# nimiq/snark-setup-operator

Hardware: NVIDIA B200
Metric: phase1_contribute_points_per_s (higher is better)
Workload: dtype u32 limbs (Montgomery, integer pipe)

## Files before the change

### snark-setup-operator_b200/csrc/curve_ops.cuh

```cuda
#pragma once
#include <type_traits>
#include "host.cuh"
#include "kernels.cuh"
#include "msm.cuh"
#include "pairing.cuh"
#include "keygen.cuh"
#include "blake2b.h"
#include <cub/device/device_radix_sort.cuh>
#include <random>

namespace sso {

struct CurveOps {
  int (*tau_tables)(Ctx& c, int si, uint64_t first_index, const uint8_t* tau, const uint8_t* const coeffs[TAU_COEFF_SLOTS],
                    uint32_t** d_table, char* err, size_t errcap);
  int (*batch_exp)(Ctx& c, int si, uint32_t group, const VecBatch& batch, uint32_t in_compressed, const uint32_t* d_table,
                   uint32_t out_compressed, uint32_t check, uint32_t* d_status, char* err, size_t errcap);
  int (*batch_exp_chunk)(Ctx& c, int si, const VecBatch& b1, const VecBatch& b2, uint32_t in_compressed, const uint32_t* d_table,
                         uint32_t out_compressed, uint32_t check, uint32_t* d_status, char* err, size_t errcap);
  int (*reencode)(Ctx& c, int si, uint32_t group, const uint8_t* d_in, uint32_t in_compressed, uint64_t n, uint8_t* d_out,
                  uint32_t out_compressed, uint32_t check, uint32_t subgroup, uint32_t* d_aff, uint32_t* d_status, char* err,
                  size_t errcap);
  int (*msm_pairs)(Ctx& c, int si, uint32_t group, const uint32_t* d_aff_a, const uint32_t* d_aff_b, uint64_t n,
                   const uint8_t seed32[32], const uint64_t* tweak, uint8_t* d_out, char* err, size_t errcap);
// ... 16 lines not shown
  int (*fft_part_tables)(Ctx& c, int si, const uint32_t* root, uint32_t squarings, uint64_t e, const uint8_t* scale, uint32_t** d_table,
                         char* err, size_t errcap);
  int (*fft_row_stage)(Ctx& c, int si, uint32_t group, const uint8_t* d_x, uint64_t rows, uint64_t row_len, uint32_t log_ns, const uint32_t* root,
                       uint32_t two_adicity, uint32_t* d_status, uint8_t* d_out, char* err, size_t errcap);
};

template <class Fr>
__global__ void k_tau_tables(const uint32_t* tau_canon, const uint32_t* coeff_canon, uint64_t first_index, uint32_t* table) {
  uint32_t tid = blockIdx.x * blockDim.x + threadIdx.x;
  if (tid < (uint32_t)TAU_TABLE_ELEMS) body_tau_tables<Fr>(tid, tau_canon, coeff_canon, first_index, table);
}

#ifndef SSO_EXP_MIN_BLOCKS
#define SSO_EXP_MIN_BLOCKS 1
#endif
#ifndef SSO_EXP_MIN_BLOCKS_G1
#define SSO_EXP_MIN_BLOCKS_G1 SSO_EXP_MIN_BLOCKS
#endif
#ifndef SSO_EXP_MIN_BLOCKS_G2
#define SSO_EXP_MIN_BLOCKS_G2 SSO_EXP_MIN_BLOCKS
#endif
#ifndef SSO_SPLIT_GROUPS
#define SSO_SPLIT_GROUPS 0
#endif
template <class G>
__global__ void __launch_bounds__(128, (G::GROUP == 0 ? SSO_EXP_MIN_BLOCKS_G1 : SSO_EXP_MIN_BLOCKS_G2)) k_batch_exp(const __grid_constant__ VecBatch batch, uint32_t in_compressed,
                                                    const uint32_t* table, uint32_t check, uint32_t* jac_out, uint32_t* status) {
  extern __shared__ __align__(16) unsigned char tree_raw[];
  block_batch_exp<G>(blockIdx.x, batch, in_compressed, table, check, jac_out, status, reinterpret_cast<typename G::F::T*>(tree_raw));
}

template <class G>
__global__ void __launch_bounds__(128, 1) k_normalize_write(const __grid_constant__ VecBatch batch, const uint32_t* jac,
                                                          uint32_t out_compressed) {
  uint32_t tid = blockIdx.x * blockDim.x + threadIdx.x;
  body_normalize_write<G>(tid, batch, jac, out_compressed);
}

template <class GC>
__global__ void __launch_bounds__(128, 1) k_subgroup_coop(uint32_t n, const uint32_t* aff, const uint8_t* pts, uint32_t* status) {
  using CO = Coop<GC::F::DEG>;
  if (!CO::lane_active()) return;
  body_subgroup_coop<GC>(blockIdx.x * ExpBlock<GC>::PPB + CO::group_in_block(), n, aff, pts, status);
}

template <class G>
__global__ void __launch_bounds__(128, 1) k_reencode(uint32_t n, const uint8_t* in, uint32_t in_compressed, uint8_t* out,
                                                   uint32_t out_compressed, uint32_t check, uint32_t subgroup, uint32_t* aff_out,
                                                   uint32_t* status) {
  uint32_t tid = blockIdx.x * blockDim.x + threadIdx.x;
  body_reencode<G>(tid, n, in, in_compressed, out, out_compressed, check, subgroup, aff_out, status);
}

#ifndef SSO_CHUNK_MIN_BLOCKS
#define SSO_CHUNK_MIN_BLOCKS 1
#endif
template <class G1, class G2>
__global__ void __launch_bounds__(128, SSO_CHUNK_MIN_BLOCKS) k_batch_exp_chunk(const __grid_constant__ VecBatch b1, const __grid_constant__ VecBatch b2,
                                                          uint32_t nb2, uint32_t in_compressed, const uint32_t* table, uint32_t check,
                                                          uint32_t* jac1, uint32_t* jac2, uint32_t* status) {
  extern __shared__ __align__(16) unsigned char tree_raw[];
  if (blockIdx.x < nb2) {
    block_batch_exp<G2>(blockIdx.x, b2, in_compressed, table, check, jac2, status, reinterpret_cast<typename G2::F::T*>(tree_raw));
  } else {
    block_batch_exp<G1>(blockIdx.x - nb2, b1, in_compressed, table, check, jac1, status, reinterpret_cast<typename G1::F::T*>(tree_raw));
  }
}
template <class G1, class G2>
__global__ void __launch_bounds__(128, 1) k_normalize_chunk(const __grid_constant__ VecBatch b1, const __grid_constant__ VecBatch b2,
                                                          uint32_t nb2, const uint32_t* jac1, const uint32_t* jac2, uint32_t out_compressed) {
  if (blockIdx.x < nb2) body_normalize_write<G2>(blockIdx.x * blockDim.x + threadIdx.x, b2, jac2, out_compressed);
  else body_normalize_write<G1>((blockIdx.x - nb2) * blockDim.x + threadIdx.x, b1, jac1, out_compressed);
}

inline int coop_g2_override() {
  const char* e = getenv("SSO_COOP_G2");
  return !e || !e[0] ? -1 : (e[0] == '0' ? 0 : 1);
}
template <class GC> inline bool coop_g2_enabled() {
  int o = coop_g2_override();
  return o < 0 ? GC::COOP_DEFAULT : o != 0;
}

template <class G1, class G2>
inline int run_batch_exp_chunk(Ctx& c, int si, const VecBatch& b1, const VecBatch& b2, uint32_t in_compressed, const uint32_t* d_table,
                               uint32_t out_compressed, uint32_t check, uint32_t* d_status, char* err, size_t errcap) {
  uint64_t n1 = b1.total, n2 = b2.total;
  if (n1 + n2 == 0) return SSO_OK;
  for (uint32_t i = 0; i < b1.nseg; i++) if (b1.seg[i].n > (1u << 24)) { set_err(err, errcap, "vector longer than 2^24 elements: split the call"); return SSO_E_ARG; }
  for (uint32_t i = 0; i < b2.nseg; i++) if (b2.seg[i].n > (1u << 24)) { set_err(err, errcap, "vector longer than 2^24 elements: split the call"); return SSO_E_ARG; }
  cudaStream_t st = c.s[si];
  uint32_t *d_jac1 = nullptr, *d_jac2 = nullptr;
  int rc;
  if ((rc = c.alloc((void**)&d_jac1, (size_t)n1 * 3 * G1::F::WORDS * 4, si))) return rc;
  if ((rc = c.alloc((void**)&d_jac2, (size_t)n2 * 3 * G2::F::WORDS * 4, si))) return rc;
  uint32_t nb2 = div_up(n2, EXP_BLOCK), nb1 = div_up(n1, EXP_BLOCK);
  constexpr size_t TREE_BYTES = 16 + 2 * EXP_BLOCK * (sizeof(typename G1::F::T) > sizeof(typename G2::F::T) ? sizeof(typename G1::F::T)
                                                                                                             : sizeof(typename G2::F::T));
  if (TREE_BYTES > 48 * 1024)
    CUDA_TRY(cudaFuncSetAttribute(k_batch_exp_chunk<G1, G2>, cudaFuncAttributeMaxDynamicSharedMemorySize, (int)TREE_BYTES));
#if SSO_SPLIT_GROUPS
  {
    const int sj = (c.s[1] && !c.aliased) ? 1 : si;
    constexpr size_t TREE1 = 16 + 2 * EXP_BLOCK * sizeof(typename G1::F::T), TREE2 = 16 + 2 * EXP_BLOCK * sizeof(typename G2::F::T);
    if (TREE1 > 48 * 1024) CUDA_TRY(cudaFuncSetAttribute(k_batch_exp<G1>, cudaFuncAttributeMaxDynamicSharedMemorySize, (int)TREE1));
    if (TREE2 > 48 * 1024) CUDA_TRY(cudaFuncSetAttribute(k_batch_exp<G2>, cudaFuncAttributeMaxDynamicSharedMemorySize, (int)TREE2));
    if (sj != si && (rc = c.fork(si, sj))) return rc;
    if (n2) {
      c.begin(PK_BATCH_EXP_G2, si, n2);
      k_batch_exp<G2><<<nb2, EXP_BLOCK, TREE2, st>>>(b2, in_compressed, d_table, check, d_jac2, d_status);
      c.end(si);
// ... 640 lines not shown
```

### snark-setup-operator_b200/csrc/curves.cuh

```cuda
#pragma once
#include "ec.cuh"
#include "coop.cuh"

namespace sso {

using Fr253 = Fp<P_r253>;
using Fq377 = Fp<P_q377>;
using Fq761 = Fp<P_q761>;
using Fq4 = Fp<P_q4>;
using Fq6 = Fp<P_q6>;

using Fq377x2 = Fp2<Fq377, SmallNR<Fq377, 5, true>>;
using Fq4x2 = Fp2<Fq4, SmallNR<Fq4, 13, false>>;
using Fq6x3 = Fp3<Fq6, SmallNR<Fq6, 11, false>>;

static constexpr bool PRIME_ORDER_bls12_377_g1 = false, PRIME_ORDER_bls12_377_g2 = false, PRIME_ORDER_bw6_761_g1 = false,
                      PRIME_ORDER_bw6_761_g2 = false, PRIME_ORDER_mnt4_753_g1 = true, PRIME_ORDER_mnt4_753_g2 = false,
                      PRIME_ORDER_mnt6_753_g1 = true, PRIME_ORDER_mnt6_753_g2 = false;
#define SSO_GROUP_COMMON(NAME, FIELD, SCALAR)                                                      \
  using F = FIELD;                                                                                  \
  using Fr = SCALAR;                                                                                \
  __device__ __forceinline__ static typename F::T coeff_b() { return F::from_const(c_##NAME##_b); } \
  __device__ __forceinline__ static const uint32_t* order() { return c_##NAME##_order; }           \
  __device__ __forceinline__ static typename F::T gen_x() { return F::from_const(c_##NAME##_gx); }  \
  __device__ __forceinline__ static typename F::T gen_y() { return F::from_const(c_##NAME##_gy); }  \
  __device__ __forceinline__ static const uint32_t* cofactor() { return c_##NAME##_cofactor; }      \
  static constexpr int COFACTOR_WORDS = COFACTOR_WORDS_##NAME;                                     \
  static constexpr bool PRIME_ORDER = PRIME_ORDER_##NAME;

struct Bls12_377_G1 {
  static constexpr bool AFFINE_TABLE = true;
  static constexpr bool HAS_GLV = true;
  using Glv = GLV_bls12_377_g1;
  static constexpr int ENDO_SUBGROUP_TEST = 1;
  static constexpr bool HAS_GLS4 = false;
  static constexpr bool HAS_GLS2 = false;
  using Endo = ENDO_bls12_377;
  static constexpr uint32_t GROUP = 0;
  SSO_GROUP_COMMON(bls12_377_g1, Fq377, Fr253)
  static constexpr bool A_IS_ZERO = true;
  __device__ __forceinline__ static F::T mul_a(const F::T&) { return F::zero(); }
  __device__ __forceinline__ static bool field_sqrt(const F::T& a, F::T& o) { return F::sqrt(a, o); }
};
struct Bls12_377_G2 {
  static constexpr float VERIFY_WEIGHT = 1.6f;
  static constexpr bool AFFINE_TABLE = true;
  static constexpr bool HAS_GLV = true;
  using Glv = GLV_bls12_377_g2;
  static constexpr int ENDO_SUBGROUP_TEST = 2;
  static constexpr bool HAS_GLS4 = true;
  static constexpr bool HAS_GLS2 = false;
  using Endo = ENDO_bls12_377;
  static constexpr uint32_t GROUP = 1;
  SSO_GROUP_COMMON(bls12_377_g2, Fq377x2, Fr253)
  static constexpr bool A_IS_ZERO = true;
  __device__ __forceinline__ static F::T mul_a(const F::T&) { return F::zero(); }
  __device__ __forceinline__ static bool field_sqrt(const F::T& a, F::T& o) { return F::sqrt(a, o); }
};
struct Bw6_761_G1 {
  static constexpr bool AFFINE_TABLE = true;
  static constexpr bool HAS_GLV = true;
  using Glv = GLV_bw6_761_g1;
  static constexpr int ENDO_SUBGROUP_TEST = 3;
  using Endo = ENDO_bw6_761;
  static constexpr bool HAS_GLS4 = false;
  static constexpr bool HAS_GLS2 = false;
  static constexpr uint32_t GROUP = 0;
  SSO_GROUP_COMMON(bw6_761_g1, Fq761, Fq377)
  static constexpr bool A_IS_ZERO = true;
  __device__ __forceinline__ static F::T mul_a(const F::T&) { return F::zero(); }
  __device__ __forceinline__ static bool field_sqrt(const F::T& a, F::T& o) { return F::sqrt(a, o); }
};
struct Bw6_761_G2 {
  static constexpr float VERIFY_WEIGHT = 1.5f;
  static constexpr bool AFFINE_TABLE = true;
  static constexpr bool HAS_GLV = true;
  using Glv = GLV_bw6_761_g2;
  static constexpr int ENDO_SUBGROUP_TEST = 0;
  static constexpr bool HAS_GLS4 = false;
  static constexpr bool HAS_GLS2 = false;
  static constexpr uint32_t GROUP = 1;
  SSO_GROUP_COMMON(bw6_761_g2, Fq761, Fq377)
  static constexpr bool A_IS_ZERO = true;
  __device__ __forceinline__ static F::T mul_a(const F::T&) { return F::zero(); }
  __device__ __forceinline__ static bool field_sqrt(const F::T& a, F::T& o) { return F::sqrt(a, o); }
};
struct Mnt4_753_G1 {
  static constexpr bool AFFINE_TABLE = true;
  static constexpr bool HAS_GLV = false;
  static constexpr int ENDO_SUBGROUP_TEST = 0;
  static constexpr bool HAS_GLS4 = false;
  static constexpr bool HAS_GLS2 = false;
  static constexpr uint32_t GROUP = 0;
  SSO_GROUP_COMMON(mnt4_753_g1, Fq4, Fq6)
  static constexpr bool A_IS_ZERO = false;
  __device__ __forceinline__ static F::T mul_a(const F::T& x) { return F::dbl(x); }
  __device__ __forceinline__ static F::T mad_a_lazy(const F::T& c, const F::T& x) { return F::mad_small_lazy(c, 2u, x); }
  __device__ __forceinline__ static bool field_sqrt(const F::T& a, F::T& o) { return F::sqrt(a, o); }
};
struct Mnt4_753_G2 {
  static constexpr float VERIFY_WEIGHT = 10.f;
  static constexpr bool AFFINE_TABLE = true;
  static constexpr bool HAS_GLV = false;
  static constexpr int ENDO_SUBGROUP_TEST = 4;
  using Endo = ENDO_mnt4_753;
  static constexpr bool HAS_GLS4 = false;
  static constexpr bool HAS_GLS2 = true;
  static constexpr uint32_t GROUP = 1;
  SSO_GROUP_COMMON(mnt4_753_g2, Fq4x2, Fq6)
  static constexpr bool A_IS_ZERO = false;
  __device__ __forceinline__ static F::T mul_a(const F::T& x) { return F::mul_small<26>(x); }
  __device__ __forceinline__ static F::T mad_a_lazy(const F::T& c, const F::T& x) { return F::mad_small_lazy(c, 26u, x); }
  __device__ __forceinline__ static bool field_sqrt(const F::T& a, F::T& o) { return F::sqrt(a, o); }
};
struct Mnt6_753_G1 {
  static constexpr bool AFFINE_TABLE = true;
  static constexpr bool HAS_GLV = false;
  static constexpr int ENDO_SUBGROUP_TEST = 0;
  static constexpr bool HAS_GLS4 = false;
  static constexpr bool HAS_GLS2 = false;
  static constexpr uint32_t GROUP = 0;
  SSO_GROUP_COMMON(mnt6_753_g1, Fq6, Fq4)
  static constexpr bool A_IS_ZERO = false;
  __device__ __forceinline__ static F::T mul_a(const F::T& x) { return F::mul_small<11>(x); }
  __device__ __forceinline__ static F::T mad_a_lazy(const F::T& c, const F::T& x) { return F::mad_small_lazy(c, 11u, x); }
  __device__ __forceinline__ static bool field_sqrt(const F::T& a, F::T& o) { return F::sqrt(a, o); }
};
struct Mnt6_753_G2 {
  static constexpr float VERIFY_WEIGHT = 20.f;
  static constexpr bool AFFINE_TABLE = false;
  static constexpr bool HAS_GLV = false;
  static constexpr int ENDO_SUBGROUP_TEST = 4;
  using Endo = ENDO_mnt6_753;
  static constexpr bool HAS_GLS4 = false;
  static constexpr bool HAS_GLS2 = true;
  static constexpr uint32_t GROUP = 1;
  SSO_GROUP_COMMON(mnt6_753_g2, Fq6x3, Fq4)
  static constexpr bool A_IS_ZERO = false;
  __device__ __forceinline__ static F::T mul_a(const F::T& x) {
    return F::mul_small<11>(F::mul_u2(x));
  }
  __device__ __forceinline__ static F::T mad_a_lazy(const F::T& c, const F::T& x) { return F::add_lazy(c, mul_a(x)); }
  __device__ __forceinline__ static bool field_sqrt(const F::T& a, F::T& o) {
#ifdef SSO_FQ3_SQRT_PLAIN
    return F::sqrt_ts<TS_q6x3>(a, o, c_q6x3_tm1h, c_q6x3_tsz);
#else
    return F::sqrt_ts_norm<TS_q6x3>(a, o, c_q6x3_tsz, ENDO_mnt6_753::w1(), ENDO_mnt6_753::w2());
#endif
  }
};

#define SSO_GROUP_COOP(NAME, PLAIN, ...)                                                            \
  using Plain = PLAIN;                                                                              \
  using F = __VA_ARGS__;                                                                            \
  __device__ __forceinline__ static typename F::T coeff_b() { return F::from_const(c_##NAME##_b); } \
  __device__ __forceinline__ static bool field_sqrt(const typename F::T&, typename F::T&) { return false; }
struct Bls12_377_G2C : Bls12_377_G2 {
  static constexpr bool COOP_DEFAULT = false;
  SSO_GROUP_COOP(bls12_377_g2, Bls12_377_G2, CFp2<Fq377, 5, true>)
  __device__ __forceinline__ static F::T mul_a(const F::T&) { return F::zero(); }
};
struct Mnt4_753_G2C : Mnt4_753_G2 {
  static constexpr bool COOP_DEFAULT = true;
  SSO_GROUP_COOP(mnt4_753_g2, Mnt4_753_G2, CFp2<Fq4, 13, false>)
  __device__ __forceinline__ static F::T mul_a(const F::T& x) { return F::mul_small<26>(x); }
  __device__ __forceinline__ static F::T mad_a_lazy(const F::T& c, const F::T& x) { return F::mad_small_lazy(c, 26u, x); }
};
#ifndef SSO_MNT6_COOP_AFFINE
#define SSO_MNT6_COOP_AFFINE 1
#endif
struct Mnt6_753_G2C : Mnt6_753_G2 {
  static constexpr bool AFFINE_TABLE = SSO_MNT6_COOP_AFFINE != 0;
  static constexpr bool COOP_DEFAULT = true;
  SSO_GROUP_COOP(mnt6_753_g2, Mnt6_753_G2, CFp3<Fq6, 11, false>)
  __device__ __forceinline__ static F::T mul_a(const F::T& x) { return F::mul_small<11>(F::mul_u2(x)); }
  __device__ __forceinline__ static F::T mad_a_lazy(const F::T& c, const F::T& x) { return F::add_lazy(c, mul_a(x)); }
};
template <class G> struct CoopOf { using type = void; };
template <> struct CoopOf<Bls12_377_G2> { using type = Bls12_377_G2C; };
template <> struct CoopOf<Mnt4_753_G2> { using type = Mnt4_753_G2C; };
template <> struct CoopOf<Mnt6_753_G2> { using type = Mnt6_753_G2C; };

enum : uint32_t { CURVE_BLS12_377 = 0, CURVE_BW6_761 = 1, CURVE_MNT4_753 = 2, CURVE_MNT6_753 = 3 };
enum : uint32_t { GROUP_G1 = 0, GROUP_G2 = 1 };

template <class Fn> inline int dispatch_group(uint32_t curve, uint32_t group, Fn&& f) {
  switch (curve * 2 + group) {
    case 0: f(Bls12_377_G1{}); return 0;
    case 1: f(Bls12_377_G2{}); return 0;
    case 2: f(Bw6_761_G1{}); return 0;
    case 3: f(Bw6_761_G2{}); return 0;
    case 4: f(Mnt4_753_G1{}); return 0;
    case 5: f(Mnt4_753_G2{}); return 0;
    case 6: f(Mnt6_753_G1{}); return 0;
    case 7: f(Mnt6_753_G2{}); return 0;
  }
  return -1;
}

}
```

### snark-setup-operator_b200/csrc/ec.cuh

```cuda
#pragma once
#include "ext.cuh"

#ifndef SSO_POINT_BY_VALUE
#define SSO_POINT_BY_VALUE 0
#endif
#ifndef SSO_LAZY_EC
#define SSO_LAZY_EC 1
#endif

namespace sso {

template <class Cfg> struct SW {
  using F = typename Cfg::F;
  using FT = typename F::T;
  struct Affine { FT x, y; bool inf; };
  struct Jac { FT X, Y, Z; };

  __device__ __forceinline__ static Jac identity() { return Jac{F::one(), F::one(), F::zero()}; }
  __device__ __forceinline__ static bool is_identity(const Jac& p) { return F::is_zero(p.Z); }
  __device__ __forceinline__ static Jac from_affine(const Affine& a) {
    if (a.inf) return identity();
    return Jac{a.x, a.y, F::one()};
  }
  __device__ __forceinline__ static Jac neg(const Jac& p) { return Jac{p.X, F::neg(p.Y), p.Z}; }

  __device__ __noinline__ static bool on_curve(const Affine& p) {
    if (p.inf) return true;
    FT rhs = F::add(F::mul(F::sqr(p.x), p.x), Cfg::coeff_b());
    if (!Cfg::A_IS_ZERO) rhs = F::add(rhs, Cfg::mul_a(p.x));
    return F::eq(F::sqr(p.y), rhs);
  }
  __device__ __forceinline__ static FT rhs(const FT& x) {
    FT r = F::add(F::mul(F::sqr(x), x), Cfg::coeff_b());
    if (!Cfg::A_IS_ZERO) r = F::add(r, Cfg::mul_a(x));
    return r;
  }

  static constexpr bool BY_VALUE = SSO_POINT_BY_VALUE && F::WORDS <= 12;
  __device__ __noinline__ static Jac dbl_val(Jac p) { return dbl_body(p); }
  __device__ __noinline__ static Jac dbl_ref(const Jac& p) { return dbl_body(p); }
  __device__ __forceinline__ static Jac dbl(const Jac& p) { if constexpr (BY_VALUE) return dbl_val(p); else return dbl_ref(p); }
  __device__ __noinline__ static Jac madd_val(Jac p, Affine q) { return madd_body(p, q); }
  __device__ __noinline__ static Jac madd_ref(const Jac& p, const Affine& q) { return madd_body(p, q); }
  __device__ __forceinline__ static Jac madd(const Jac& p, const Affine& q) { if constexpr (BY_VALUE) return madd_val(p, q); else return madd_ref(p, q); }
  __device__ __noinline__ static Jac add_val(Jac p, Jac q) { return add_body(p, q); }
  __device__ __noinline__ static Jac add_ref(const Jac& p, const Jac& q) { return add_body(p, q); }
  __device__ __forceinline__ static Jac add(const Jac& p, const Jac& q) { if constexpr (BY_VALUE) return add_val(p, q); else return add_ref(p, q); }

  __device__ __forceinline__ static Jac dbl_lazy_body(const Jac& p) {
    Jac r;
    constexpr bool TRADE = !F::SQR_CHEAPER;
    if constexpr (Cfg::A_IS_ZERO) {
      FT A = F::sqr(p.X);
      FT B = F::sqr(p.Y);
      FT D, C8;
      if constexpr (TRADE) {
        FT X2 = F::add_lazy(p.X, p.X);
        D = F::mul(F::add_lazy(X2, X2), B);
        C8 = F::dbl(F::sqr(F::add_lazy(B, B)));
      } else {
        FT C = F::sqr(B);
        D = F::dbl(F::sub(F::sub(F::sqr(F::add_lazy(p.X, B)), A), C));
        C8 = F::dbl(F::dbl(F::dbl(C)));
      }
      FT E = F::add_lazy(F::add_lazy(A, A), A);
      r.Z = F::mul(F::add_lazy(p.Y, p.Y), p.Z);
      r.X = F::sub(F::sqr(E), F::dbl(D));
      r.Y = F::sub(F::mul(E, F::sub_lazy(D, r.X)), C8);
    } else {
      FT XX = F::sqr(p.X);
      FT YY = F::sqr(p.Y);
      FT ZZ = F::sqr(p.Z);
      FT S, Y8;
      if constexpr (TRADE) {
        FT X2 = F::add_lazy(p.X, p.X);
        S = F::mul(F::add_lazy(X2, X2), YY);
        r.Z = F::mul(F::add_lazy(p.Y, p.Y), p.Z);
        Y8 = F::dbl(F::sqr(F::add_lazy(YY, YY)));
      } else {
        FT YYYY = F::sqr(YY);
        S = F::dbl(F::sub(F::sub(F::sqr(F::add_lazy(p.X, YY)), XX), YYYY));
        r.Z = F::sub(F::sub(F::sqr(F::add_lazy(p.Y, p.Z)), YY), ZZ);
        Y8 = F::dbl(F::dbl(F::dbl(YYYY)));
      }
      FT M = Cfg::mad_a_lazy(F::add_lazy(F::add_lazy(XX, XX), XX), F::sqr(ZZ));
      r.X = F::sub(F::sqr(M), F::dbl(S));
      r.Y = F::sub(F::mul(M, F::sub_lazy(S, r.X)), Y8);
    }
    return r;
  }

  __device__ __forceinline__ static Jac dbl_body(const Jac& p) {
    if constexpr (SSO_LAZY_EC && F::LAZY_OK) return dbl_lazy_body(p);
    Jac r;
    if (Cfg::A_IS_ZERO) {
      FT A = F::sqr(p.X);
      FT B = F::sqr(p.Y);
      FT C = F::sqr(B);
      FT D = F::sub(F::sub(F::sqr(F::add(p.X, B)), A), C);
      D = F::dbl(D);
      FT E = F::add(F::dbl(A), A);
      FT Fq = F::sqr(E);
      r.Z = F::dbl(F::mul(p.Y, p.Z));
      r.X = F::sub(Fq, F::dbl(D));
      FT C8 = F::dbl(F::dbl(F::dbl(C)));
      r.Y = F::sub(F::mul(E, F::sub(D, r.X)), C8);
    } else {
      FT XX = F::sqr(p.X);
      FT YY = F::sqr(p.Y);
      FT YYYY = F::sqr(YY);
      FT ZZ = F::sqr(p.Z);
      FT S = F::sub(F::sub(F::sqr(F::add(p.X, YY)), XX), YYYY);
      S = F::dbl(S);
      FT M = F::add(F::add(F::dbl(XX), XX), Cfg::mul_a(F::sqr(ZZ)));
      r.Z = F::sub(F::sub(F::sqr(F::add(p.Y, p.Z)), YY), ZZ);
      r.X = F::sub(F::sqr(M), F::dbl(S));
      FT Y8 = F::dbl(F::dbl(F::dbl(YYYY)));
      r.Y = F::sub(F::mul(M, F::sub(S, r.X)), Y8);
    }
    return r;
  }

  __device__ __forceinline__ static Jac madd_body(const Jac& p, const Affine& q) {
    if (q.inf) return p;
    if (is_identity(p)) return Jac{q.x, q.y, F::one()};
    FT Z1Z1 = F::sqr(p.Z);
    FT U2 = F::mul(q.x, Z1Z1);
    FT S2 = F::mul(F::mul(q.y, p.Z), Z1Z1);
    FT H = F::sub(U2, p.X);
    FT rr = F::sub(S2, p.Y);
    if (F::is_zero(H)) {
      if (F::is_zero(rr)) return dbl(p);
      return identity();
    }
    if constexpr (SSO_LAZY_EC && F::LAZY_OK) {
      FT r2 = F::add_lazy(rr, rr);
      FT HH = F::sqr(H);
      FT HH2 = F::add_lazy(HH, HH);
      FT I = F::add_lazy(HH2, HH2);
      FT J = F::mul(H, I);
      FT V = F::mul(p.X, I);
      Jac r;
      r.X = F::sub(F::sub(F::sqr(r2), J), F::dbl(V));
      r.Y = F::sub(F::mul(r2, F::sub_lazy(V, r.X)), F::mul(F::add_lazy(p.Y, p.Y), J));
      if constexpr (!F::SQR_CHEAPER) r.Z = F::mul(F::add_lazy(p.Z, p.Z), H);
      else r.Z = F::sub(F::sub(F::sqr(F::add_lazy(p.Z, H)), Z1Z1), HH);
      return r;
    }
    rr = F::dbl(rr);
    FT HH = F::sqr(H);
    FT I = F::dbl(F::dbl(HH));
    FT J = F::mul(H, I);
    FT V = F::mul(p.X, I);
    Jac r;
    r.X = F::sub(F::sub(F::sqr(rr), J), F::dbl(V));
    r.Y = F::sub(F::mul(rr, F::sub(V, r.X)), F::dbl(F::mul(p.Y, J)));
    r.Z = F::sub(F::sub(F::sqr(F::add(p.Z, H)), Z1Z1), HH);
    return r;
  }

  __device__ __forceinline__ static Jac add_body(const Jac& p, const Jac& q) {
    if (is_identity(p)) return q;
    if (is_identity(q)) return p;
    FT Z1Z1 = F::sqr(p.Z);
    FT Z2Z2 = F::sqr(q.Z);
    FT U1 = F::mul(p.X, Z2Z2);
    FT U2 = F::mul(q.X, Z1Z1);
    FT S1 = F::mul(F::mul(p.Y, q.Z), Z2Z2);
    FT S2 = F::mul(F::mul(q.Y, p.Z), Z1Z1);
    FT H = F::sub(U2, U1);
    FT rr = F::sub(S2, S1);
    if (F::is_zero(H)) {
      if (F::is_zero(rr)) return dbl(p);
      return identity();
    }
    rr = F::dbl(rr);
    FT I = F::sqr(F::dbl(H));
    FT J = F::mul(H, I);
    FT V = F::mul(U1, I);
    Jac r;
    r.X = F::sub(F::sub(F::sqr(rr), J), F::dbl(V));
    r.Y = F::sub(F::mul(rr, F::sub(V, r.X)), F::dbl(F::mul(S1, J)));
    r.Z = F::mul(F::sub(F::sub(F::sqr(F::add(p.Z, q.Z)), Z1Z1), Z2Z2), H);
    return r;
  }

  template <int KL, int NW>
  __device__ __forceinline__ static void bias_scalar(const uint32_t* k, uint32_t* kb) {
    constexpr int BL = (4 * NW + 31) / 32;
    uint32_t carry = 0;
#pragma unroll
    for (int i = 0; i < BL; i++) {
      uint32_t ki = i < KL ? k[i] : 0u;
      int lo = 32 * i, hi = 32 * i + 32;
      uint32_t c = 0x88888888u;
      if (4 * NW < hi) c = (4 * NW <= lo) ? 0u : (0x88888888u & ((1u << (4 * NW - lo)) - 1u));
      uint64_t s = (uint64_t)ki + c + carry;
      kb[i] = (uint32_t)s;
      carry = (uint32_t)(s >> 32);
// ... 76 lines not shown
    mul_low<KW, KW, KW>(c1, GLV::b1(), t); limbs_sub<KW>(k2, k2, t);
    mul_low<KW, KW, KW>(c2, GLV::b2(), t); limbs_sub<KW>(k2, k2, t);
    uint32_t z[KW];
#pragma unroll
    for (int i = 0; i < KW; i++) z[i] = 0u;
    neg1 = (k1[KW - 1] >> 31) != 0;
    neg2 = (k2[KW - 1] >> 31) != 0;
    if (neg1) limbs_sub<KW>(k1, z, k1);
    if (neg2) limbs_sub<KW>(k2, z, k2);
  }
  __device__ __forceinline__ static FT mul_beta(const FT& x, const uint32_t* beta) {
    typename F::Base::T b = F::Base::from_const(beta);
    if constexpr (F::DEG == 1) return F::mul(x, b);
    else return F::mul_base(x, b);
  }

  template <class GLV, int KL>
  __device__ __forceinline__ static Jac scalar_mul_glv(const Affine& base, const uint32_t* k) {
    constexpr int KW = GLV::KW;
    constexpr int NW = (GLV::KBITS + 2 + 3) / 4;
    constexpr int BL = (4 * NW + 31) / 32;
    static_assert(BL >= KW, "window count must cover the half-size scalars");
    if (base.inf) return identity();
    uint32_t k1[KW], k2[KW], kb1[BL], kb2[BL];
    bool neg1, neg2;
    glv_split<GLV, KL>(k, k1, k2, neg1, neg2);
    bias_scalar<KW, NW>(k1, kb1);
    bias_scalar<KW, NW>(k2, kb2);
    Jac tab[8];
    build_table(base, tab);
    Jac acc = identity();
#pragma unroll 1
    for (int w = NW - 1; w >= 0; w--) {
      if (w != NW - 1) {
#pragma unroll 1
        for (int d = 0; d < 4; d++) acc = dbl(acc);
      }
      int d1 = digit(kb1, w), d2 = digit(kb2, w);
      if (d1 != 0) {
        Jac q = tab[(d1 < 0 ? -d1 : d1) - 1];
        if ((d1 < 0) != neg1) q.Y = F::neg(q.Y);
        acc = add(acc, q);
      }
      if (d2 != 0) {
        Jac q = tab[(d2 < 0 ? -d2 : d2) - 1];
        q.X = mul_beta(q.X, GLV::beta());
        if ((d2 < 0) != neg2) q.Y = F::neg(q.Y);
        acc = add(acc, q);
      }
    }
    return acc;
  }

  template <bool GLVMODE, int KW_, int NW_> struct Staged {
    static constexpr int NW = NW_;
    static constexpr int BL = (4 * NW + 31) / 32;
    Jac tab[8];
    uint32_t kb1[BL], kb2[BL];
    bool neg1, neg2, active, affine;
  };

  template <class ST>
  __device__ __forceinline__ static FT staged_table(ST& st, const Affine& base) {
    st.active = !base.inf;
    st.affine = false;
    if (!st.active) return F::one();
    build_table(base, st.tab);
    if constexpr (!Cfg::AFFINE_TABLE) return F::one();
    FT prod = st.tab[1].Z;
    bool ok = !F::is_zero(prod);
#pragma unroll 1
    for (int i = 2; i < 8; i++) {
      ok = ok && !F::is_zero(st.tab[i].Z);
      prod = F::mul(prod, st.tab[i].Z);
    }
    st.affine = ok;
    return ok ? prod : F::one();
  }
  template <class ST>
  __device__ __forceinline__ static void staged_normalise(ST& st, const FT& zinv_all) {
    if (!st.active || !st.affine) return;
    FT pre[8];
    pre[1] = st.tab[1].Z;
#pragma unroll 1
    for (int i = 2; i < 8; i++) pre[i] = F::mul(pre[i - 1], st.tab[i].Z);
    FT inv = zinv_all;
#pragma unroll 1
    for (int i = 7; i >= 1; i--) {
      FT zi = i > 1 ? F::mul(inv, pre[i - 1]) : inv;
      if (i > 1) inv = F::mul(inv, st.tab[i].Z);
      FT zi2 = F::sqr(zi);
      st.tab[i].X = F::mul(st.tab[i].X, zi2);
      st.tab[i].Y = F::mul(st.tab[i].Y, F::mul(zi2, zi));
    }
  }
  template <class ST>
  __device__ __forceinline__ static Jac staged_add(const ST& st, const Jac& acc, int dgt, bool neg, const uint32_t* beta) {
    int idx = (dgt < 0 ? -dgt : dgt) - 1;
    bool flip = (dgt < 0) != neg;
    if (st.affine) {
      Affine q{st.tab[idx].X, st.tab[idx].Y, false};
      if (beta) q.x = mul_beta(q.x, beta);
      if (flip) q.y = F::neg(q.y);
      return madd(acc, q);
    }
    Jac q = st.tab[idx];
    if (beta) q.X = mul_beta(q.X, beta);
    if (flip) q.Y = F::neg(q.Y);
    return add(acc, q);
  }
  __device__ __forceinline__ static FT endo_frob(const FT& a) {
    using E = typename Cfg::Endo;
    if constexpr (F::DEG == 2) { return F::conj(a); }
    else { return F::frob_w(a, E::w1(), E::w2()); }
  }
  template <int KL>
  __device__ __forceinline__ static void gls2_split(const uint32_t* k, uint32_t* k0, uint32_t* k1) {
    using E = typename Cfg::Endo;
    constexpr int KW = E::GLS_KW, GW = E::GLS_GW;
    static_assert(KL == 24 && KW <= 12, "768-bit Barrett shift");
    uint32_t prod[KL + GW];
    mul_low<KL, GW, KL + GW>(k, E::recip(), prod);
    uint32_t q[KW + 1];
#pragma unroll
    for (int i = 0; i <= KW; i++) q[i] = KL + i < KL + GW ? prod[KL + i] : 0u;
    uint32_t t[KL], rem[KL];
    mul_low<KW, KW, KL>(q, E::tm1(), t);
    limbs_sub<KL>(rem, k, t);
    uint32_t mu[KL], one[KW + 1];
#pragma unroll
    for (int i = 0; i < KL; i++) mu[i] = i < KW ? E::tm1()[i] : 0u;
#pragma unroll
    for (int i = 0; i <= KW; i++) one[i] = i == 0 ? 1u : 0u;
    for (int it = 0; it < 2; it++) {
      uint32_t d[KL];
      if (limbs_sub<KL>(d, rem, mu) == 0) {
#pragma unroll
        for (int i = 0; i < KL; i++) rem[i] = d[i];
        limbs_add<KW + 1>(q, q, one);
      }
    }
#pragma unroll
    for (int i = 0; i < KW; i++) { k0[i] = rem[i]; k1[i] = q[i]; }
  }
  template <class ST>
  __device__ __forceinline__ static Jac staged_add_psi(const ST& st, const Jac& acc, int dgt, bool neg) {
    using E = typename Cfg::Endo;
    using B = typename F::Base;
    int idx = (dgt < 0 ? -dgt : dgt) - 1;
    bool flip = (dgt < 0) != neg;
    FT x = F::mul_base(endo_frob(st.tab[idx].X), B::from_const(E::cx()));
    FT y = F::mul_base(endo_frob(st.tab[idx].Y), B::from_const(E::cy()));
    if (flip) y = F::neg(y);
    if (st.affine) return madd(acc, Affine{x, y, false});
    return add(acc, Jac{x, y, endo_frob(st.tab[idx].Z)});
  }

  template <class ST>
  __device__ __forceinline__ static Jac staged_loop(const ST& st, const uint32_t* beta) {
    Jac acc = identity();
    if (!st.active) return acc;
#pragma unroll 1
    for (int w = ST::NW - 1; w >= 0; w--) {
      if (w != ST::NW - 1) {
#pragma unroll 1
        for (int d = 0; d < 4; d++) acc = dbl(acc);
      }
      int d1 = digit(st.kb1, w);
      if (d1 != 0) acc = staged_add(st, acc, d1, st.neg1, nullptr);
      if constexpr (Cfg::HAS_GLS2) {
        int d2 = digit(st.kb2, w);
        if (d2 != 0) acc = staged_add_psi(st, acc, d2, st.neg2);
      } else if (beta) {
        int d2 = digit(st.kb2, w);
        if (d2 != 0) acc = staged_add(st, acc, d2, st.neg2, beta);
      }
    }
    return acc;
  }

  template <int NW_> struct Staged4 {
    static constexpr int NW = NW_;
    static constexpr int BL = (4 * NW + 31) / 32;
    Jac tab[8];
    uint32_t kb[4][BL];
    bool active, affine;
  };
  template <int KL>
  __device__ __forceinline__ static void gls4_split(const uint32_t* k, uint32_t kd[4][2]) {
    constexpr unsigned long long X = Cfg::Endo::X;
    unsigned long long n[4];
#pragma unroll
    for (int i = 0; i < 4; i++) n[i] = (2 * i < KL ? (unsigned long long)k[2 * i] : 0ull) | (2 * i + 1 < KL ? (unsigned long long)k[2 * i + 1] << 32 : 0ull);
#pragma unroll 1
    for (int d = 0; d < 4; d++) {
      unsigned long long rem = 0;
#pragma unroll 1
      for (int i = 3; i >= 0; i--) {
        unsigned __int128 cur = ((unsigned __int128)rem << 64) | n[i];
        n[i] = (unsigned long long)(cur / X);
        rem = (unsigned long long)(cur % X);
      }
      kd[d][0] = (uint32_t)rem;
      kd[d][1] = (uint32_t)(rem >> 32);
    }
  }
  template <class ST>
  __device__ __forceinline__ static Jac staged_add4(const ST& st, const Jac& acc, int dgt, int j) {
    using B = typename F::Base;
    using E = typename Cfg::Endo;
    int idx = (dgt < 0 ? -dgt : dgt) - 1;
    bool flip = dgt < 0;
    Jac q = st.tab[idx];
    if (j == 1) {
      q.X = F::mul_base(F::conj(q.X), B::from_const(E::psi_cx()));
      q.Y = F::mul_base(F::conj(q.Y), B::from_const(E::psi_cy()));
      q.Z = F::conj(q.Z);
    } else if (j == 2) {
      q.X = F::mul_base(q.X, B::from_const(E::psi_omega()));
      flip = !flip;
    } else if (j == 3) {
      q.X = F::neg(F::conj(q.X));
      q.Y = F::mul_base(F::conj(q.Y), B::from_const(E::psi_cy()));
      q.Z = F::conj(q.Z);
      flip = !flip;
    }
    if (flip) q.Y = F::neg(q.Y);
    if (st.affine) return madd(acc, Affine{q.X, q.Y, false});
    return add(acc, q);
  }
  template <class ST>
  __device__ __forceinline__ static Jac staged_loop4(const ST& st) {
    Jac acc = identity();
    if (!st.active) return acc;
#pragma unroll 1
    for (int w = ST::NW - 1; w >= 0; w--) {
      if (w != ST::NW - 1) {
#pragma unroll 1
        for (int d = 0; d < 4; d++) acc = dbl(acc);
      }
#pragma unroll 1
      for (int j = 0; j < 4; j++) {
        int dg = digit(st.kb[j], w);
        if (dg != 0) acc = staged_add4(st, acc, dg, j);
      }
    }
    return acc;
  }

  static constexpr int NAF_MAX_WORDS = 48;
#ifndef SSO_NO_NAF
#define SSO_NO_NAF 0
#endif
  __device__ __noinline__ static Jac mul_const(const Affine& base, const uint32_t* e, int nwords) {
    int weight = 0, bitlen = 0;
    for (int i = 0; i < nwords; i++) {
      weight += __popc(e[i]);
      if (e[i]) bitlen = 32 * i + 32 - __clz(e[i]);
    }
    if (SSO_NO_NAF || nwords > NAF_MAX_WORDS || weight * 100 <= 30 * bitlen + 500 || base.inf) {
      Jac acc = identity();
      for (int i = nwords * 32 - 1; i >= 0; i--) {
        acc = dbl(acc);
        if ((e[i >> 5] >> (i & 31)) & 1) acc = madd(acc, base);
      }
      return acc;
    }
    uint32_t k[NAF_MAX_WORDS + 1];
    for (int i = 0; i <= NAF_MAX_WORDS; i++) k[i] = i < nwords ? e[i] : 0u;
    signed char dig[32 * NAF_MAX_WORDS + 2];
    int nd = 0, top = nwords;
    for (;;) {
      while (top > 0 && k[top] == 0) top--;
      if (top == 0 && k[0] == 0) break;
      int d = 0;
      if (k[0] & 1u) {
        d = (int)(k[0] & 15u);
        if (d >= 8) d -= 16;
        if (d > 0) {
          uint32_t b = (uint32_t)d;
          for (int i = 0; i <= top && b; i++) { uint32_t o = k[i]; k[i] = o - b; b = o < b ? 1u : 0u; }
        } else {
// ... 138 lines not shown
```

### snark-setup-operator_b200/csrc/kernels.cuh

```cuda
#pragma once
#include <type_traits>
#include "curves.cuh"

namespace sso {

enum : uint32_t { CHECK_NO = 0, CHECK_NONZERO = 1, CHECK_FULL = 2 };
enum : uint32_t { ST_OK = 0, ST_NONCANONICAL = 1, ST_BAD_FLAGS = 2, ST_NOT_ON_CURVE = 3, ST_ZERO_POINT = 4,
                  ST_NOT_IN_SUBGROUP = 5 };

__device__ __forceinline__ void report(uint32_t* status, uint32_t code, uint32_t index, uint32_t vec = 0) {
#ifdef SSO_HOST_EMUL
  if (status[0] == 0) { status[0] = code; status[1] = index; status[2] = vec; }
#else
  if (atomicCAS(&status[0], 0u, code) == 0u) { status[1] = index; status[2] = vec; }
#endif
}

static constexpr int TAU_COEFF_SLOTS = 3;
static constexpr int TAU_TABLE_ELEMS = 769 + TAU_COEFF_SLOTS;

struct VecSeg {
  const uint8_t* in;
  uint8_t* out;
  uint32_t n;
// ... 58 lines not shown
#define SSO_EXP_BLOCK 128
#endif
static constexpr int EXP_BLOCK = SSO_EXP_BLOCK;

template <class F> __device__ __forceinline__ void tree_up(typename F::T* tree, int n, int t) {
  if (t < n) tree[n + t] = F::mul(tree[2 * (n + t)], tree[2 * (n + t) + 1]);
}
template <class F> __device__ __forceinline__ void tree_down(typename F::T* tree, int n, int t) {
  if (t < n) {
    int k = n + t;
    typename F::T l = tree[2 * k], r = tree[2 * k + 1], pinv = tree[k];
    tree[2 * k] = F::mul(pinv, r);
    tree[2 * k + 1] = F::mul(pinv, l);
  }
}
#ifndef SSO_HOST_EMUL
template <class F> __device__ __forceinline__ void block_batch_inverse(typename F::T* tree, int t) {
  for (int n = EXP_BLOCK / 2; n >= 1; n >>= 1) { __syncthreads(); tree_up<F>(tree, n, t); }
  __syncthreads();
  if (t == 0) tree[1] = F::inv(tree[1]);
  for (int n = 1; n < EXP_BLOCK; n <<= 1) { __syncthreads(); tree_down<F>(tree, n, t); }
  __syncthreads();
}
#else
template <class F> inline void block_batch_inverse_all(typename F::T* tree) {
  for (int n = EXP_BLOCK / 2; n >= 1; n >>= 1) for (int t = 0; t < n; t++) tree_up<F>(tree, n, t);
  tree[1] = F::inv(tree[1]);
  for (int n = 1; n < EXP_BLOCK; n <<= 1) for (int t = 0; t < n; t++) tree_down<F>(tree, n, t);
}
#endif

template <class G> struct ExpTypes {
  using C = SW<G>;
  using Fr = typename G::Fr;
  static constexpr bool GLS4 = G::HAS_GLS4;
  static constexpr bool GLS2 = G::HAS_GLS2;
  static constexpr bool GLV = G::HAS_GLV && !GLS4;
  static constexpr int KBITS = [] { if constexpr (G::HAS_GLS4) return 64; else if constexpr (G::HAS_GLS2) return (int)G::Endo::GLS_KBITS; else if constexpr (G::HAS_GLV) return (int)G::Glv::KBITS; else return (int)G::Fr::P::BITS; }();
  static constexpr int KW = [] { if constexpr (G::HAS_GLS4) return 2; else if constexpr (G::HAS_GLS2) return (int)G::Endo::GLS_KW; else if constexpr (G::HAS_GLV) return (int)G::Glv::KW; else return (int)G::Fr::L; }();
  static constexpr int NW = (KBITS + 2 + 3) / 4;
  using State = std::conditional_t<GLS4, typename C::template Staged4<NW>, typename C::template Staged<GLV || GLS2, KW, NW>>;
};

template <class G, bool TWIDDLE = false>
__device__ __forceinline__ typename G::F::T exp_stage_a(uint32_t tid, const VecBatch& b, uint32_t in_compressed, const uint32_t* table,
                                                        uint32_t check, uint32_t* status, typename ExpTypes<G>::State& st,
                                                        const uint8_t* staged_src = nullptr, uint32_t tw_mask = 0, uint32_t tw_shift = 0) {
  using C = SW<G>;
  using F = typename G::F;
  using Fr = typename G::Fr;
  using ET = ExpTypes<G>;
  uint32_t sidx, j;
  st.active = false;
  st.affine = false;
  if (!locate(b, tid, sidx, j)) return F::one();
  const VecSeg& sg = b.seg[sidx];
  typename C::Affine p;
  const uint8_t* src = staged_src ? staged_src : sg.in + (size_t)j * (in_compressed ? C::SIZE_C : C::SIZE_U);
  uint32_t dst;
  if constexpr (F::COOP != 0) dst = C::read_uncompressed(src, p);
  else dst = in_compressed ? C::read_compressed(src, p) : C::read_uncompressed(src, p);
  if (dst != C::DESER_OK) { report(status, dst, j, sidx); p.inf = true; }
  if (check != CHECK_NO && dst == C::DESER_OK) {
    if (p.inf) report(status, ST_ZERO_POINT, j, sidx);
    else if (check == CHECK_FULL && !in_compressed && !C::on_curve(p)) { report(status, ST_NOT_ON_CURVE, j, sidx); p.inf = true; }
  }
  uint32_t k[Fr::L];
  if constexpr (TWIDDLE) {
    scalar_for_index<Fr>(table, (j >> tw_shift) & tw_mask, tw_mask + 1, false, 0, k);
  } else if (sg.mode == 0) {
    scalar_for_index<Fr>(table, j, sg.n, sg.has_coeff != 0, sg.coeff_slot, k);
  } else {
    typename Fr::T s = Fr::from_mont(Fr::load(table + (size_t)(769 + sg.coeff_slot) * Fr::L, 1));
#pragma unroll
    for (int i = 0; i < Fr::L; i++) k[i] = s.v[i];
  }
  if constexpr (ET::GLS4) {
    uint32_t kd[4][2];
    C::template gls4_split<Fr::L>(k, kd);
#pragma unroll
    for (int d = 0; d < 4; d++) C::template bias_scalar<2, ET::NW>(kd[d], st.kb[d]);
  } else if constexpr (ET::GLS2) {
    uint32_t k0[ET::KW], k1[ET::KW];
    C::template gls2_split<Fr::L>(k, k0, k1);
    st.neg1 = false;
    st.neg2 = G::Endo::TM1_NEG;
    C::template bias_scalar<ET::KW, ET::NW>(k0, st.kb1);
    C::template bias_scalar<ET::KW, ET::NW>(k1, st.kb2);
  } else if constexpr (ET::GLV) {
    uint32_t k1[ET::KW], k2[ET::KW];
    C::template glv_split<typename G::Glv, Fr::L>(k, k1, k2, st.neg1, st.neg2);
    C::template bias_scalar<ET::KW, ET::NW>(k1, st.kb1);
    C::template bias_scalar<ET::KW, ET::NW>(k2, st.kb2);
  } else {
    st.neg1 = st.neg2 = false;
    C::template bias_scalar<Fr::L, ET::NW>(k, st.kb1);
  }
  return C::staged_table(st, p);
}

template <class G>
__device__ __forceinline__ void exp_stage_c(uint32_t tid, const VecBatch& b, typename ExpTypes<G>::State& st,
                                            const typename G::F::T& zinv, uint32_t* jac_out) {
  using C = SW<G>;
  using F = typename G::F;
  if (tid >= b.total) return;
  C::staged_normalise(st, zinv);
// ... 314 lines not shown
```

Measured before the change: 9.712 million.

## Always normalise staged tables via prefix/suffix products and raise G2 chunk occupancy

Replaces the per-call conditional affine table path with a Table struct that records zero-Z entries as an infinity bitmask. It precomputes each entry's partner product with prefix and suffix scans, so normalisation needs one multiply per entry instead of recomputing prefix products. The 'affine' flag disappears and the mixed-add path is always taken when the curve uses affine tables. Doubling and addition formulas are reordered to shorten live ranges. The BLS12-377 G2 chunk kernel now requests 3 blocks per SM through a per-group launch bound, which may force register spills.

```diff
diff --git a/snark-setup-operator_b200/csrc/curve_ops.cuh b/snark-setup-operator_b200/csrc/curve_ops.cuh
--- a/snark-setup-operator_b200/csrc/curve_ops.cuh
+++ b/snark-setup-operator_b200/csrc/curve_ops.cuh
@@ -92,11 +92,8 @@
   body_reencode<G>(tid, n, in, in_compressed, out, out_compressed, check, subgroup, aff_out, status);
 }
 
-#ifndef SSO_CHUNK_MIN_BLOCKS
-#define SSO_CHUNK_MIN_BLOCKS 1
-#endif
 template <class G1, class G2>
-__global__ void __launch_bounds__(128, SSO_CHUNK_MIN_BLOCKS) k_batch_exp_chunk(const __grid_constant__ VecBatch b1, const __grid_constant__ VecBatch b2,
+__global__ void __launch_bounds__(128, G2::CHUNK_MIN_BLOCKS) k_batch_exp_chunk(const __grid_constant__ VecBatch b1, const __grid_constant__ VecBatch b2,
                                                           uint32_t nb2, uint32_t in_compressed, const uint32_t* table, uint32_t check,
                                                           uint32_t* jac1, uint32_t* jac2, uint32_t* status) {
   extern __shared__ __align__(16) unsigned char tree_raw[];
diff --git a/snark-setup-operator_b200/csrc/curves.cuh b/snark-setup-operator_b200/csrc/curves.cuh
--- a/snark-setup-operator_b200/csrc/curves.cuh
+++ b/snark-setup-operator_b200/csrc/curves.cuh
@@ -52,6 +52,7 @@
   static constexpr bool HAS_GLS2 = false;
   using Endo = ENDO_bls12_377;
   static constexpr uint32_t GROUP = 1;
+  static constexpr int CHUNK_MIN_BLOCKS = 3;
   SSO_GROUP_COMMON(bls12_377_g2, Fq377x2, Fr253)
   static constexpr bool A_IS_ZERO = true;
   __device__ __forceinline__ static F::T mul_a(const F::T&) { return F::zero(); }
@@ -80,6 +81,7 @@
   static constexpr bool HAS_GLS4 = false;
   static constexpr bool HAS_GLS2 = false;
   static constexpr uint32_t GROUP = 1;
+  static constexpr int CHUNK_MIN_BLOCKS = 1;
   SSO_GROUP_COMMON(bw6_761_g2, Fq761, Fq377)
   static constexpr bool A_IS_ZERO = true;
   __device__ __forceinline__ static F::T mul_a(const F::T&) { return F::zero(); }
@@ -107,6 +109,7 @@
   static constexpr bool HAS_GLS4 = false;
   static constexpr bool HAS_GLS2 = true;
   static constexpr uint32_t GROUP = 1;
+  static constexpr int CHUNK_MIN_BLOCKS = 1;
   SSO_GROUP_COMMON(mnt4_753_g2, Fq4x2, Fq6)
   static constexpr bool A_IS_ZERO = false;
   __device__ __forceinline__ static F::T mul_a(const F::T& x) { return F::mul_small<26>(x); }
@@ -135,6 +138,7 @@
   static constexpr bool HAS_GLS4 = false;
   static constexpr bool HAS_GLS2 = true;
   static constexpr uint32_t GROUP = 1;
+  static constexpr int CHUNK_MIN_BLOCKS = 1;
   SSO_GROUP_COMMON(mnt6_753_g2, Fq6x3, Fq4)
   static constexpr bool A_IS_ZERO = false;
   __device__ __forceinline__ static F::T mul_a(const F::T& x) {
@@ -157,6 +161,7 @@
   __device__ __forceinline__ static bool field_sqrt(const typename F::T&, typename F::T&) { return false; }
 struct Bls12_377_G2C : Bls12_377_G2 {
   static constexpr bool COOP_DEFAULT = false;
+  static constexpr int CHUNK_MIN_BLOCKS = 1;
   SSO_GROUP_COOP(bls12_377_g2, Bls12_377_G2, CFp2<Fq377, 5, true>)
   __device__ __forceinline__ static F::T mul_a(const F::T&) { return F::zero(); }
 };
diff --git a/snark-setup-operator_b200/csrc/ec.cuh b/snark-setup-operator_b200/csrc/ec.cuh
--- a/snark-setup-operator_b200/csrc/ec.cuh
+++ b/snark-setup-operator_b200/csrc/ec.cuh
@@ -51,20 +51,22 @@
     Jac r;
     constexpr bool TRADE = !F::SQR_CHEAPER;
     if constexpr (Cfg::A_IS_ZERO) {
-      FT A = F::sqr(p.X);
+      r.Z = F::mul(F::add_lazy(p.Y, p.Y), p.Z);
       FT B = F::sqr(p.Y);
       FT D, C8;
+      FT A;
       if constexpr (TRADE) {
+        A = F::sqr(p.X);
         FT X2 = F::add_lazy(p.X, p.X);
         D = F::mul(F::add_lazy(X2, X2), B);
         C8 = F::dbl(F::sqr(F::add_lazy(B, B)));
       } else {
         FT C = F::sqr(B);
+        A = F::sqr(p.X);
         D = F::dbl(F::sub(F::sub(F::sqr(F::add_lazy(p.X, B)), A), C));
         C8 = F::dbl(F::dbl(F::dbl(C)));
       }
       FT E = F::add_lazy(F::add_lazy(A, A), A);
-      r.Z = F::mul(F::add_lazy(p.Y, p.Y), p.Z);
       r.X = F::sub(F::sqr(E), F::dbl(D));
       r.Y = F::sub(F::mul(E, F::sub_lazy(D, r.X)), C8);
     } else {
@@ -134,17 +136,18 @@
       return identity();
     }
     if constexpr (SSO_LAZY_EC && F::LAZY_OK) {
-      FT r2 = F::add_lazy(rr, rr);
       FT HH = F::sqr(H);
+      Jac r;
+      if constexpr (!F::SQR_CHEAPER) r.Z = F::mul(F::add_lazy(p.Z, p.Z), H);
+      else r.Z = F::sub(F::sub(F::sqr(F::add_lazy(p.Z, H)), Z1Z1), HH);
       FT HH2 = F::add_lazy(HH, HH);
       FT I = F::add_lazy(HH2, HH2);
       FT J = F::mul(H, I);
       FT V = F::mul(p.X, I);
-      Jac r;
+      FT r2 = F::add_lazy(rr, rr);
       r.X = F::sub(F::sub(F::sqr(r2), J), F::dbl(V));
-      r.Y = F::sub(F::mul(r2, F::sub_lazy(V, r.X)), F::mul(F::add_lazy(p.Y, p.Y), J));
-      if constexpr (!F::SQR_CHEAPER) r.Z = F::mul(F::add_lazy(p.Z, p.Z), H);
-      else r.Z = F::sub(F::sub(F::sqr(F::add_lazy(p.Z, H)), Z1Z1), HH);
+      FT W = F::mul(F::add_lazy(p.Y, p.Y), J);
+      r.Y = F::sub(F::mul(r2, F::sub_lazy(V, r.X)), W);
       return r;
     }
     rr = F::dbl(rr);
@@ -327,62 +330,66 @@
     return acc;
   }
 
+  struct Table {
+    Jac e[8];
+    uint32_t inf;
+  };
   template <bool GLVMODE, int KW_, int NW_> struct Staged {
     static constexpr int NW = NW_;
     static constexpr int BL = (4 * NW + 31) / 32;
-    Jac tab[8];
+    Table tab;
     uint32_t kb1[BL], kb2[BL];
-    bool neg1, neg2, active, affine;
+    bool neg1, neg2, active;
   };
 
   template <class ST>
   __device__ __forceinline__ static FT staged_table(ST& st, const Affine& base) {
+    Table& t = st.tab;
     st.active = !base.inf;
-    st.affine = false;
+    t.inf = 0;
     if (!st.active) return F::one();
-    build_table(base, st.tab);
+    build_table(base, t.e);
     if constexpr (!Cfg::AFFINE_TABLE) return F::one();
-    FT prod = st.tab[1].Z;
-    bool ok = !F::is_zero(prod);
-#pragma unroll 1
-    for (int i = 2; i < 8; i++) {
-      ok = ok && !F::is_zero(st.tab[i].Z);
-      prod = F::mul(prod, st.tab[i].Z);
-    }
-    st.affine = ok;
-    return ok ? prod : F::one();
+    FT z[8];
+#pragma unroll 1
+    for (int i = 1; i < 8; i++) {
+      z[i] = t.e[i].Z;
+      if (F::is_zero(z[i])) { t.inf |= 1u << i; z[i] = F::one(); }
+    }
+    FT d = z[1];
+#pragma unroll 1
+    for (int i = 2; i < 8; i++) { t.e[i].Z = d; d = F::mul(d, z[i]); }
+    FT suf = z[7];
+#pragma unroll 1
+    for (int i = 6; i >= 2; i--) { t.e[i].Z = F::mul(t.e[i].Z, suf); suf = F::mul(suf, z[i]); }
+    t.e[1].Z = suf;
+    return d;
   }
   template <class ST>
   __device__ __forceinline__ static void staged_normalise(ST& st, const FT& zinv_all) {
-    if (!st.active || !st.affine) return;
-    FT pre[8];
-    pre[1] = st.tab[1].Z;
-#pragma unroll 1
-    for (int i = 2; i < 8; i++) pre[i] = F::mul(pre[i - 1], st.tab[i].Z);
-    FT inv = zinv_all;
-#pragma unroll 1
-    for (int i = 7; i >= 1; i--) {
-      FT zi = i > 1 ? F::mul(inv, pre[i - 1]) : inv;
-      if (i > 1) inv = F::mul(inv, st.tab[i].Z);
+    if constexpr (!Cfg::AFFINE_TABLE) return;
+    if (!st.active) return;
+    Table& t = st.tab;
+#pragma unroll 1
+    for (int i = 1; i < 8; i++) {
+      FT zi = F::mul(zinv_all, t.e[i].Z);
       FT zi2 = F::sqr(zi);
-      st.tab[i].X = F::mul(st.tab[i].X, zi2);
-      st.tab[i].Y = F::mul(st.tab[i].Y, F::mul(zi2, zi));
-    }
+      t.e[i].X = F::mul(t.e[i].X, zi2);
+      t.e[i].Y = F::mul(t.e[i].Y, F::mul(zi2, zi));
+    }
+  }
+  __device__ __forceinline__ static Jac table_add(const Table& t, const Jac& acc, int idx, const FT& x, const FT& y, const FT& z) {
+    if constexpr (Cfg::AFFINE_TABLE) return madd(acc, Affine{x, y, ((t.inf >> idx) & 1u) != 0});
+    else return add(acc, Jac{x, y, z});
   }
   template <class ST>
   __device__ __forceinline__ static Jac staged_add(const ST& st, const Jac& acc, int dgt, bool neg, const uint32_t* beta) {
     int idx = (dgt < 0 ? -dgt : dgt) - 1;
     bool flip = (dgt < 0) != neg;
-    if (st.affine) {
-      Affine q{st.tab[idx].X, st.tab[idx].Y, false};
-      if (beta) q.x = mul_beta(q.x, beta);
-      if (flip) q.y = F::neg(q.y);
-      return madd(acc, q);
-    }
-    Jac q = st.tab[idx];
-    if (beta) q.X = mul_beta(q.X, beta);
-    if (flip) q.Y = F::neg(q.Y);
-    return add(acc, q);
+    FT x = st.tab.e[idx].X, y = st.tab.e[idx].Y;
+    if (beta) x = mul_beta(x, beta);
+    if (flip) y = F::neg(y);
+    return table_add(st.tab, acc, idx, x, y, st.tab.e[idx].Z);
   }
   __device__ __forceinline__ static FT endo_frob(const FT& a) {
     using E = typename Cfg::Endo;
@@ -424,11 +431,10 @@
     using B = typename F::Base;
     int idx = (dgt < 0 ? -dgt : dgt) - 1;
     bool flip = (dgt < 0) != neg;
-    FT x = F::mul_base(endo_frob(st.tab[idx].X), B::from_const(E::cx()));
-    FT y = F::mul_base(endo_frob(st.tab[idx].Y), B::from_const(E::cy()));
+    FT x = F::mul_base(endo_frob(st.tab.e[idx].X), B::from_const(E::cx()));
+    FT y = F::mul_base(endo_frob(st.tab.e[idx].Y), B::from_const(E::cy()));
     if (flip) y = F::neg(y);
-    if (st.affine) return madd(acc, Affine{x, y, false});
-    return add(acc, Jac{x, y, endo_frob(st.tab[idx].Z)});
+    return table_add(st.tab, acc, idx, x, y, Cfg::AFFINE_TABLE ? st.tab.e[idx].Z : endo_frob(st.tab.e[idx].Z));
   }
 
   template <class ST>
@@ -457,9 +463,9 @@
   template <int NW_> struct Staged4 {
     static constexpr int NW = NW_;
     static constexpr int BL = (4 * NW + 31) / 32;
-    Jac tab[8];
+    Table tab;
     uint32_t kb[4][BL];
-    bool active, affine;
+    bool active;
   };
   template <int KL>
   __device__ __forceinline__ static void gls4_split(const uint32_t* k, uint32_t kd[4][2]) {
@@ -486,7 +492,7 @@
     using E = typename Cfg::Endo;
     int idx = (dgt < 0 ? -dgt : dgt) - 1;
     bool flip = dgt < 0;
-    Jac q = st.tab[idx];
+    Jac q = st.tab.e[idx];
     if (j == 1) {
       q.X = F::mul_base(F::conj(q.X), B::from_const(E::psi_cx()));
       q.Y = F::mul_base(F::conj(q.Y), B::from_const(E::psi_cy()));
@@ -501,8 +507,7 @@
       flip = !flip;
     }
     if (flip) q.Y = F::neg(q.Y);
-    if (st.affine) return madd(acc, Affine{q.X, q.Y, false});
-    return add(acc, q);
+    return table_add(st.tab, acc, idx, q.X, q.Y, q.Z);
   }
   template <class ST>
   __device__ __forceinline__ static Jac staged_loop4(const ST& st) {
diff --git a/snark-setup-operator_b200/csrc/kernels.cuh b/snark-setup-operator_b200/csrc/kernels.cuh
--- a/snark-setup-operator_b200/csrc/kernels.cuh
+++ b/snark-setup-operator_b200/csrc/kernels.cuh
@@ -134,7 +134,6 @@
   using ET = ExpTypes<G>;
   uint32_t sidx, j;
   st.active = false;
-  st.affine = false;
   if (!locate(b, tid, sidx, j)) return F::one();
   const VecSeg& sg = b.seg[sidx];
   typename C::Affine p;
```

Result: faster. 10.40 million (median of 6 runs) (+7.1%).
